# dfm/emcee

Hardware: AMD Instinct MI355X
Metric: walker-updates/sec (whole node), 64-dim correlated Gaussian, StretchMove a=2 (higher is better)
Workload: dtype f64

## Files before the change

emcee_amd/_lib.py:

```python
import ctypes as C
import os

import numpy as np

HERE = os.path.dirname(os.path.abspath(__file__))
LIB_PATH = os.path.join(HERE, "libemx.so")

TARGET_HOST, TARGET_ISO, TARGET_DIAG, TARGET_DENSE, TARGET_ROSENBROCK, TARGET_BOX, TARGET_CALLBACK = range(7)
TARGET_FUSED_USER = 8
TARGET_FUSED_PT = 9
TARGET_FUSED_ENSEMBLE = 10
MOVE_STRETCH, MOVE_DE, MOVE_SNOOKER, MOVE_GAUSS = range(4)
MOVE_WALK, MOVE_KDE = 5, 6
KDE_BW_SCOTT, KDE_BW_SILVERMAN, KDE_BW_SCALAR = range(3)
GAUSS_VECTOR, GAUSS_RANDOM, GAUSS_SEQUENTIAL = range(3)
RNG_INPUTS, RNG_MT19937, RNG_PHILOX = range(3)
EXCHANGE_ALLGATHER, EXCHANGE_PULL, EXCHANGE_DIRECT, EXCHANGE_LOGPROB, EXCHANGE_REPLAY = range(5)


class MoveDesc(C.Structure):
    _fields_ = [("kind", C.c_int32), ("nsplits", C.c_int32), ("randomize_split", C.c_int32), ("reserved", C.c_int32),
                ("a", C.c_double), ("sigma", C.c_double), ("g0", C.c_double), ("gammas", C.c_double)]


# ... 123 lines not shown
    "emx_logprob_finish": (C.c_int, [_P, C.c_int32]),
    "emx_replay_begin": (C.c_int, [_P, C.c_int32, C.POINTER(C.c_int64)]),
    "emx_replay_finish": (C.c_int, [_P, C.c_int32]),
    "emx_replay_exchange": (C.c_int, [_P, C.c_int32]),
    "emx_replica_pack": (C.c_int, [_P, C.POINTER(C.c_int64)]),
    "emx_replica_unpack": (C.c_int, [_P]),
    "emx_direct_export": (C.c_int, [_P, _u8p]),
    "emx_direct_import": (C.c_int, [_P, _u8p]),
    "emx_direct_attach": (C.c_int, [_P, C.POINTER(C.c_void_p), C.POINTER(C.c_void_p)]),
    "emx_direct_halfstep": (C.c_int, [_P, C.c_int32, C.c_int32]),
    "emx_fft_load": (C.c_int, [C.c_char_p]),
    "emx_autocorr": (C.c_int, [_P, C.c_int64, C.c_int64, C.c_double, _dp, _ip, C.POINTER(C.c_int64)]),
    "emx_walkers_independent": (C.c_int, [C.c_int32, _dp, C.c_int64, C.c_int32, C.POINTER(C.c_int32), C.POINTER(C.c_double)]),
    "emx_walkers_independent_resident": (C.c_int, [C.c_void_p, C.POINTER(C.c_int32), C.POINTER(C.c_double)]),
    "emx_host_pull_capacity": (C.c_int64, [C.c_int64, C.c_int32, C.c_int32, C.c_int32]),
    "emx_comm_load": (C.c_int, [C.c_char_p]),
    "emx_comm_get_unique_id": (C.c_int, [_u8p]),
    "emx_comm_init": (C.c_int, [_P, C.c_int32, C.c_int32, _u8p]),
    "emx_comm_destroy": (C.c_int, [_P]),
    "emx_comm_count": (C.c_int, [_P, C.POINTER(C.c_int32)]),
    "emx_pipeline_stats": (C.c_int, [_P, _dp, C.POINTER(C.c_int64), C.POINTER(C.c_int32)]),
    "emx_pipeline_handovers": (C.c_int, [_P, C.POINTER(C.c_int64), C.POINTER(C.c_int64)]),
    "emx_persist_info": (C.c_int, [_P, C.POINTER(C.c_int64)]),
    "emx_mtdev_info": (C.c_int, [_P, C.POINTER(C.c_int64)]),
    "emx_mtdev_debug": (C.c_int, [_P, C.c_int32, C.c_int64, C.c_void_p, C.c_int64]),
    "emx_mtdev_tok_stats": (C.c_int, [_P, C.POINTER(C.c_int64)]),
    "emx_persist_local_launches": (C.c_int, [_P, C.POINTER(C.c_int64)]),
    "emx_host_mt_jump": (C.c_int, [_u32p, C.c_uint64, C.c_int32, _u32p]),
    "emx_host_persist_shape": (C.c_int, [C.c_int64, C.c_int32, C.c_int32, C.POINTER(C.c_int32), C.POINTER(C.c_int32)]),
    "emx_timer_start": (C.c_int, [_P]),
    "emx_timer_stop": (C.c_int, [_P, C.POINTER(C.c_float)]),
    "emx_profile_enable": (C.c_int, [_P, C.c_int32]),
    "emx_profile_read": (C.c_int, [_P, _f32p, C.POINTER(C.c_int32)]),
    "emx_mt_create": (_P, [_u32p, C.c_int32, C.c_int32, C.c_double]),
    "emx_mt_destroy": (None, [_P]),
    "emx_mt_get_state": (None, [_P, _u32p, C.POINTER(C.c_int32), C.POINTER(C.c_int32), C.POINTER(C.c_double)]),
    "emx_mt_random_sample": (None, [_P, C.c_int64, _dp]),
    "emx_mt_randint": (None, [_P, C.c_uint64, C.c_int64, _i64p]),
    "emx_mt_randn": (None, [_P, C.c_int64, _dp]),
    "emx_mt_shuffle_labels": (None, [_P, C.c_int64, C.c_int32, _ip]),
    "emx_mt_choice_cdf": (C.c_int32, [_P, _dp, C.c_int32]),
    "emx_host_plan_mt": (C.c_int, [_P, C.c_int64, C.c_int32, C.POINTER(MoveDesc), _ip, _ip, _ip, _ip, _ip, _dp, _dp]),
    "emx_host_plan_mt_stream": (C.c_int, [_P, C.c_int64, C.c_int32, C.c_int32, C.POINTER(MoveDesc), _dp, C.c_int64, C.c_int32, C.c_int32,
                                          _P, _P, _P, _P, _P, _P, _P, C.POINTER(C.c_double)]),
    "emx_host_split_draws": (C.c_int, [_P, C.c_int64, C.POINTER(MoveDesc), _ip, _ip, C.c_int32, _ip, _ip, _ip, _dp]),
    "emx_host_plan_philox": (C.c_int, [C.c_uint64, C.c_uint64, C.c_int64, C.POINTER(MoveDesc), _ip, _ip, _ip, _ip, _ip, _dp, _dp]),
# ... 103 lines not shown
```

emcee_amd/csrc/emx.hip:

```cpp
#include <hip/hip_runtime.h>

#include <dlfcn.h>

#include <algorithm>
#include <chrono>
#include <cmath>
#include <cstdint>
#include <cstdio>
#include <cstring>
#include <deque>
#include <mutex>
#include <string>
#include <type_traits>
#include <vector>

#include "../../include/emx.h"
#include "emx_fused_ensemble.hpp"
#include "emx_fused_ensemble_data.hpp"
#include "emx_internal.hpp"
#include "emx_kernels.hpp"
#include "emx_launch.hpp"
#include "emx_mtdev.hpp"
#include "emx_mtjump.hpp"
#include "emx_mtpipe.hpp"
// ... 340 lines not shown
    int64_t tune_persist_slab_local_max = 4096;
    int64_t call_steps = 1;
    int64_t tune_persist_exact = 1;
    int64_t tune_persist_valu = 1;
    int64_t tune_persist_local_max = 8192;
    int64_t tune_slab = 1;
    int64_t tune_slab_skew = 1;
    int64_t tune_mt_device = 1;
    int64_t tune_mt_device_min = 147456;
    int64_t tune_mt_lookahead = 2;
    int64_t tune_mt_tok_wshift = 11, tune_mt_tok_tail = 2048;
    int64_t mtdev_steps_total = 0, mtdev_starts = 0;
    bool mtdev_defer_release = false;
    int64_t mtdev_release_pending = -1;
    MtDevStats mtdev_stats_last;
    int ring_pos = 0;
    struct Prepared {
        int move, S, slot;
        bool lean;
        int gcol;
        uint64_t step;
        NativeArgs nat;
        double cursor_before;
    };
    std::deque<Prepared> prepared;
    int64_t prep_hint = 1;
    std::vector<uint8_t> labels_scratch;
    struct Cur {
        bool active = false;
        int move = 0, S = 2, slot = 0;
        bool store = false;
        bool native = false;
        bool lean = false;
        bool devplan = false;
        int gcol = 0;
        std::vector<int32_t> off;
        NativeArgs nat{};
    } cur;
    double *chain = nullptr, *chain_lp = nullptr;
    int64_t cap = 0, stored = 0, proposals = 0;
    EnsSummary* summary = nullptr;
    RhatScratch* rhat = nullptr;
    int64_t tune_summary_compact = 1;
    int64_t tune_hist_chunk_rows = 0;
    double *qout = nullptr, *fout = nullptr, *newlp = nullptr;
    double* tp1_full = nullptr;
    double *evalX = nullptr, *evallp = nullptr;
    double* wk_work = nullptr;
// ... 90 lines not shown
    std::vector<hipEvent_t> prof;
    int prof_max = 0, prof_n = 0;
    std::string err;
    emx_fused_ensemble_data_fn fused_data_fn = nullptr;
    int64_t fused_ndata = 0;
    int64_t tune_fused_data_rows = 0;
};

static void graph_invalidate(emx_ctx* c);
static void apply_env_tuning(emx_ctx* c);
static int pipe_stop(emx_ctx* c);
#define PIPE_STOP(ctx)                        \
    do {                                      \
        const int _rps = pipe_stop(ctx);      \
        if (_rps) return _rps;                \
    } while (0)
static void direct_detach(emx_ctx* c);
static int direct_ensure(emx_ctx* c);
static void exchange_free(emx_ctx* c);
static int replay_ensure(emx_ctx* c);
static int flags_ensure(emx_ctx* c);
static int persist_settle(emx_ctx* c);
static hipError_t wait_stream(hipStream_t s);

static void drop_prepared(emx_ctx* c) {
    for (auto it = c->prepared.rbegin(); it != c->prepared.rend(); ++it)
        if (it->move < (int)c->moves.size() && c->moves[it->move].kind == EMX_MOVE_GAUSS) c->moves[it->move].gammas = it->cursor_before;
    c->prepared.clear();
}

#define FAIL(ctx, code, ...)                         \
    do {                                             \
        char _b[512];                                \
        snprintf(_b, sizeof(_b), __VA_ARGS__);       \
        if (ctx) (ctx)->err = _b; else g_err = _b;   \
        return (code);                               \
    } while (0)

#define HIPOK(ctx, expr)                                                                          \
    do {                                                                                          \
        hipError_t _e = (expr);                                                                   \
        if (_e != hipSuccess) FAIL(ctx, -2, "%s failed: %s (%s:%d)", #expr, hipGetErrorString(_e), __FILE__, __LINE__); \
    } while (0)

#define NEED(ctx, cond, ...)               \
    do {                                   \
// ... 732 lines not shown
}

static void apply_env_tuning(emx_ctx* c) {
    const char* e = getenv("EMX_TUNE");
    if (!e || !*e) return;
    std::string s(e);
    size_t pos = 0;
    while (pos < s.size()) {
        size_t end = s.find(',', pos);
        if (end == std::string::npos) end = s.size();
        const std::string kv = s.substr(pos, end - pos);
        const size_t eq = kv.find('=');
        if (eq != std::string::npos) emx_set_tuning(c, kv.substr(0, eq).c_str(), atoll(kv.c_str() + eq + 1));
        pos = end + 1;
    }
}

int emx_destroy(emx_ctx* c) {
    if (!c) return 0;
    pipe_stop(c);
    c->plog.clear();
    hipSetDevice(c->device);
    if (c->stream) hipStreamSynchronize(c->stream);
    if (c->comm && g_rccl.CommDestroy) g_rccl.CommDestroy(c->comm), c->comm = nullptr;
    if (c->status_host) hipHostFree(c->status_host);
    if (c->xfer_host) hipHostFree(c->xfer_host);
    for (int k = 0; k < 2; ++k) {
        if (c->bounce[k]) hipHostFree(c->bounce[k]);
        if (c->bounce_ev[k]) hipEventDestroy(c->bounce_ev[k]);
    }
    void* ptrs[] = {c->X, c->lp, c->acc, c->acc_count, c->iota, c->qout, c->fout, c->newlp, c->evalX, c->wk_work,
                    c->evallp, c->tp0, c->tp1, c->tp1_full, c->chain, c->chain_lp, c->own_shard_bufs ? c->sendbuf : nullptr,
                    c->own_shard_bufs ? c->gathered : nullptr};
    for (void* p : ptrs)
        if (p) hipFree(p);
    for (double* s : c->snap)
        if (s) hipFree(s);
    for (double* s : c->snap_blobs)
        if (s) hipFree(s);
    for (double* s : {c->blobs, c->evalblobs, c->blob_plane})
        if (s) hipFree(s);
    emx_internal_ens_summary_release(c->summary);
    emx_internal_rhat_release(c->rhat);

    for (auto& s : c->ring) {
        if (s.order) hipFree(s.order);
// ... 64 lines not shown
            const hipError_t e = hipStreamQuery(s);
            if (e != hipErrorNotReady) return e;
            if ((it & 63) == 63 && std::chrono::steady_clock::now() - t0 > std::chrono::milliseconds(2)) break;
        }
    }
    return hipStreamSynchronize(s);
}

static hipError_t wait_event(hipEvent_t ev) {
    if (g_spin_sync) {
        const auto t0 = std::chrono::steady_clock::now();
        for (int it = 0;; ++it) {
            const hipError_t e = hipEventQuery(ev);
            if (e != hipErrorNotReady) return e;
            if ((it & 63) == 63 && std::chrono::steady_clock::now() - t0 > std::chrono::milliseconds(2)) break;
        }
    }
    return hipEventSynchronize(ev);
}

int emx_sync(emx_ctx* c) {
    HIPOK(c, hipSetDevice(c->device));
    HIPOK(c, wait_stream(c->stream));
    return persist_settle(c);
}

int emx_status(emx_ctx* c, uint32_t* bits) {
    HIPOK(c, wait_stream(c->stream));
    {
        const int rcs = persist_settle(c);
        if (rcs) return rcs;
    }
    uint32_t b = 0;
    for (int k = 0; k < 6; ++k)
        if (__atomic_exchange_n(&c->status_host[k], 0u, __ATOMIC_ACQ_REL)) b |= 1u << k;
    if (b & ST_EXCHANGE_TIMEOUT) c->direct_dead = true;
    if (b & ST_EXCHANGE_TIMEOUT) c->persist_grid = 0;
    *bits = b;
    return 0;
}

int emx_set_tuning(emx_ctx* c, const char* key, int64_t v) {
    if (!strcmp(key, "spw")) {
        c->tune_spw = v;
        return 0;
    }
    if (!strcmp(key, "phase_clock")) {
// ... 153 lines not shown
        PIPE_STOP(c);
        c->tune_persist_exact = v ? 1 : 0;
        return 0;
    }
    if (!strcmp(key, "persist_exact_max_walkers")) {
        PIPE_STOP(c);
        c->tune_persist_exact_max = v;
        return 0;
    }
    if (!strcmp(key, "persist_exact_steps")) {
        c->tune_persist_exact_steps = std::max<int64_t>(1, std::min<int64_t>(v, 16));
        return 0;
    }
    if (!strcmp(key, "fetch_blocks")) {
        c->tune_fetch_blocks = std::max<int64_t>(0, std::min<int64_t>(v, 65536));
        return 0;
    }
    if (!strcmp(key, "fetch_avoid")) {
        c->tune_fetch_avoid = v ? 1 : 0;
        return 0;
    }
    if (!strcmp(key, "test_fetch_delay_us")) {
        c->tune_fetch_delay_us = std::max<int64_t>(0, std::min<int64_t>(v, 100000));
        return 0;
    }
    if (!strcmp(key, "persist_span")) {
        c->tune_persist_span = v ? 1 : 0;
        return 0;
    }
    if (!strcmp(key, "persist_mix")) {
        c->tune_persist_mix = v ? 1 : 0;
        return 0;
    }
    if (!strcmp(key, "persist_valu")) {
        c->tune_persist_valu = v ? 1 : 0;
        return 0;
    }
    if (!strcmp(key, "persist_local_max_walkers")) {
        c->tune_persist_local_max = v;
        return 0;
    }
    if (!strcmp(key, "persist_gauss_wpb")) {
        c->tune_persist_gauss_wpb = (v == 1 || v == 2 || v == 4 || v == 8) ? v : 0;
        return 0;
    }
    if (!strcmp(key, "persist_test_skew")) {
// ... 1065 lines not shown
    if (any_raw) hipLaunchKernelGGL(k_plan_raw_batch, dim3((unsigned)F.pieces_x, (unsigned)F.n), dim3(256), 0, c->up_stream, RB);
    HIPOK(c, hipGetLastError());
    hipEvent_t& ev = c->pipe_batch_ev[c->pipe_batch_n & 3];
    if (!ev) HIPOK(c, hipEventCreateWithFlags(&ev, hipEventDisableTiming));
    c->pipe_batch_n++;
    HIPOK(c, hipEventRecord(ev, c->up_stream));
    HIPOK(c, hipStreamWaitEvent(c->stream, ev, 0));
    for (auto& d : c->pipe_deferred) {
        c->ring[d.second].uploaded_ref = ev;
    }
    c->pipe_deferred.clear();
    return 0;
}

int emx_step_begin(emx_ctx* c, int32_t store, int32_t* move_out, int32_t* S_out) {
    return step_begin_impl(c, store, -1, move_out, S_out);
}

int emx_step_begin_with(emx_ctx* c, int32_t store, int32_t move_index, int32_t* S_out) {
    NEED(c, move_index >= 0 && move_index < (int)c->moves.size(), "bad move index");
    return step_begin_impl(c, store, move_index, nullptr, S_out);
}

static int native_prepare_batch(emx_ctx* c, uint64_t first_step, int nb, int forced_move, hipStream_t st) {
    const int nm = (int)c->moves.size();
    NativeBatchArgs B{};
    B.N = (int32_t)c->N;
    B.D = c->D;
    B.nb = nb;
    B.lean = (c->target != EMX_TARGET_HOST && c->world == 1 && !c->sendbuf && !c->comm && !c->tune_full_plan) ? 1 : 0;
    B.ablate = (int32_t)(c->tune_ablate >> 8);
    bool only_stretch = true;
    for (int b = 0; b < nb; ++b) {
        const uint64_t step = first_step + (uint64_t)b;
        const int mi = forced_move >= 0 ? forced_move : philox_move_choice(c->ph_seed, step, c->cdf.data(), nm);
        const emx_move_desc& m = c->moves[mi];
        only_stretch = only_stretch && m.kind == EMX_MOVE_STRETCH;
        emx_ctx::PlanSlot* ps;
        int rc = acquire_slot(c, &ps, false);
        if (rc) return rc;
        emx_ctx::Prepared pr{};
        pr.move = mi;
        pr.S = m.nsplits;
        pr.slot = c->ring_pos;
        pr.step = step;
        pr.nat.seed = c->ph_seed;
        pr.nat.step = step;
        pr.nat.pk = make_perm_key((uint64_t)c->N, c->ph_seed, step);
        pr.cursor_before = m.gammas;
        pr.lean = B.lean != 0;
        if (m.kind == EMX_MOVE_GAUSS) {
            B.gmode[b] = m.reserved;
            B.gcol[b] = (int32_t)((int64_t)m.gammas % c->D);
            pr.gcol = B.gcol[b];
            if (m.reserved == EMX_GAUSS_SEQUENTIAL) c->moves[mi].gammas = (double)(((int64_t)m.gammas + 1) % c->D);
        }
        c->prepared.push_back(pr);
        B.nat[b] = pr.nat;
        B.order[b] = ps->order;
        B.p0[b] = ps->p0;
        B.p1[b] = ps->p1;
        B.p2[b] = ps->p2;
        B.s0[b] = ps->s0;
        B.uacc[b] = ps->uacc;
        B.logu[b] = ps->logu;
        B.fac[b] = ps->fac;
        B.a[b] = m.a;
        B.sigma[b] = m.sigma;
        B.g0[b] = m.g0;
        B.move[b] = m.kind;
        B.S[b] = m.nsplits;
    }
    if (only_stretch && B.lean && !B.ablate && !B.desc)
        hipLaunchKernelGGL(k_native_plan_batch_stretch, dim3((unsigned)((c->N + 255) / 256), (unsigned)nb), dim3(256), 0, st, B);
    else
        hipLaunchKernelGGL(k_native_plan_batch, dim3((unsigned)((c->N + 255) / 256), (unsigned)nb), dim3(256), 0, st, B);
    HIPOK(c, hipGetLastError());
    return 0;
}

static int step_begin_impl(emx_ctx* c, int32_t store, int32_t forced_move, int32_t* move_out, int32_t* S_out) {
    HIPOK(c, hipSetDevice(c->device));
    NEED(c, !c->cur.active, "emx_step_begin: previous step not ended");
    if (store) NEED(c, c->stored < c->cap, "chain capacity exhausted (call emx_chain_config)");
    auto& cur = c->cur;
    cur.store = store != 0;
    cur.native = false;
    cur.devplan = false;
    const int nm = (int)c->moves.size();
    const bool devp = forced_move < 0 && mtdev_eligible(c);
    if (c->mtdev && !devp) {
        const int rcm = mtdev_stop(c);
        if (rcm) return rcm;
    }
    if (c->pipe && (devp || forced_move >= 0 || !pipe_eligible(c))) PIPE_STOP(c);
    if (devp) {
        if (!c->mtdev) {
            int rc0 = mtdev_start(c);
            if (rc0) return rc0;
        }
        int rc = mtdev_take(c);
        if (rc) return rc;
    } else if (c->rng_mode == EMX_RNG_MT19937 && forced_move < 0 && (c->pipe || ((c->N >= 8192 || persist_exact_ok(c)) && pipe_eligible(c)))) {
        if (!c->pipe) {
            int rc0 = pipe_start(c);
            if (rc0) return rc0;
        }
// ... 948 lines not shown
    const size_t lds = dense_lds_bytes(c->Dp, wpb);
    hipEvent_t e0 = nullptr, e1 = nullptr;
    const bool prof = c->prof_max > 0 && c->prof_n < c->prof_max;
    if (prof) {
        e0 = c->prof[2 * c->prof_n];
        e1 = c->prof[2 * c->prof_n + 1];
        HIPOK(c, hipEventRecord(e0, c->stream));
    }
    const hipError_t e = launch_hot_persist_gauss(c->Dp / 16, grid, block, lds, c->stream, P);
    if (e != hipSuccess) FAIL(c, -2, "persistent Gaussian launch failed: %s", hipGetErrorString(e));
    if (prof) {
        HIPOK(c, hipEventRecord(e1, c->stream));
        c->prof_n++;
    }
    c->persist_launches++;
    c->persist_halfsteps += steps;
    *done = steps;
    return 0;
}

static std::mutex g_persist_mu;
static hipEvent_t g_persist_ev[MAX_DEVICES] = {};
static const emx_ctx* g_persist_last[MAX_DEVICES] = {};

static int run_persist(emx_ctx* c, int64_t i0, int64_t total, int32_t thin_by, int32_t store, int64_t* done) {
    *done = 0;
    if (__atomic_load_n(&c->status_host[3], __ATOMIC_ACQUIRE)) {
        const int rcs = persist_settle(c);
        if (rcs) return rcs;
        if (__atomic_load_n(&c->status_host[3], __ATOMIC_ACQUIRE)) {
            c->persist_grid = 0;
            FAIL(c, -8, "persistent kernel: a device-wide barrier timed out in the middle of a launch; read emx_status, "
                        "or turn the persistent path off with tuning \"persist\" = 0");
        }
        return 0;
    }
    if (c->plog.size() >= 4096) {
        if (hipStreamQuery(c->stream) == hipSuccess && !__atomic_load_n(&c->status_host[3], __ATOMIC_ACQUIRE)) {
            c->plog.clear();
        } else if (c->plog.size() >= 65536) {
            const int rcs = persist_settle(c);
            if (rcs) return rcs;
        }
    }
    if (!c->persist_bar) {
        HIPOK(c, hipMalloc((void**)&c->persist_bar, PERSIST_BAR_WORDS * sizeof(unsigned)));
// ... 22 lines not shown
    } undefer2{c};
    c->mtdev_defer_release = devp;
    c->mtdev_release_pending = -1;
    struct Undefer {
        emx_ctx* c;
        ~Undefer() { c->mtdev_defer_release = false; }
    } undefer{c};
    emx_ctx::PersistLog lg{};
    lg.ph_step = c->ph_step;
    lg.i0 = i0;
    lg.stored0 = c->stored;
    lg.proposals0 = c->proposals;
    lg.thin_by = thin_by;
    lg.store = store;
    if (mtmode && !devp) {
        lg.pipe_step0 = c->pipe ? c->pipe_taken : 0;
        lg.pipe_id = c->pipe;
    }
    int launch_move = -1;
    int launch_S = 2;
    bool launch_local = false;
    bool launch_mix = false;
    double launch_gammas = 0.0;
    int batches_touched = (!mtmode && !c->prepared.empty() && c->prepared.front().step == c->ph_step) ? 1 : 0;
    while (i0 + steps < total) {
        if (!mtmode && (c->prepared.empty() || c->prepared.front().step != c->ph_step)) {
            if (batches_touched >= 2) break;
            ++batches_touched;
        }
        int next_move = -1;
        if (steps > 0 && !mtmode)
            next_move = !c->prepared.empty() ? c->prepared.front().move : philox_move_choice(c->ph_seed, c->ph_step, c->cdf.data(), (int)c->moves.size());
        if (steps > 0 && mtmode && !devp && c->moves.size() > 1) {
            PipeStepInfo peek;
            if (!c->pipe || !c->pipe->wait_ready(c->pipe_taken, peek, pipe_poll, c))
                FAIL(c, -7, "exact-mode plan pipeline stopped before step %lld", (long long)c->pipe_taken);
            next_move = peek.move;
        }
        int need = launch_S;
        if (launch_mix && next_move >= 0) need = c->moves[next_move].nsplits;
        if (n + need > (int)std::min<int64_t>(PERSIST_MAX_ITERS, std::max<int64_t>(4, c->tune_persist_max_halfsteps))) break;
        if (devp) {
            if (steps > 0 && c->mtdev && c->mtdev_taken % MTDEV_BATCH == 0) break;
        } else if (mtmode) {
            if (steps >= std::min<int64_t>(c->tune_persist_exact_steps, c->pipe_nsinks / 2)) break;
            if (steps > 0 && next_move >= 0) {
                if (!launch_mix && c->moves[next_move].kind != launch_move) break;
                if (!launch_mix && launch_move == EMX_MOVE_SNOOKER && c->moves[next_move].gammas != launch_gammas) break;
                if (launch_mix && !persist_mix_member(c->moves[next_move])) break;
                if (!persist_move_ok(c, c->moves[next_move])) break;
            }
// ... 1 lines not shown
            if (steps > 0 && c->prepared.empty() && !c->tune_persist_span) break;
            if (steps > 0 && !launch_mix && c->moves[next_move].kind != launch_move) break;
            if (steps > 0 && !launch_mix && launch_move == EMX_MOVE_SNOOKER && c->moves[next_move].gammas != launch_gammas) break;
            if (steps > 0 && launch_mix && !persist_mix_member(c->moves[next_move])) break;
            if (steps > 0 && !persist_move_ok(c, c->moves[next_move])) break;
        }
        c->prep_hint = NATIVE_BATCH_MAX;
        const int st = store && ((i0 + steps + 1) % thin_by == 0);
        int mvi, S;
        int rc = emx_step_begin(c, st, &mvi, &S);
        if (rc) return rc;
        if (launch_move < 0) {
            launch_move = c->moves[mvi].kind;
            launch_gammas = c->moves[mvi].gammas;
            launch_S = S;
            launch_local = persist_local_ok(c, c->moves[mvi]);
            c->persist_wpb = launch_local ? persist_shape_local_of(c->N, S, c->num_cu) : persist_shape(c, S);
            if (persist_mix_ok(c) && (launch_move == EMX_MOVE_DE || launch_move == EMX_MOVE_SNOOKER)) {
                launch_mix = true;
                launch_local = persist_mix_local(c);
                c->persist_wpb = launch_local ? persist_shape_local_of(c->N, 2, c->num_cu) : persist_shape(c, 2);
            }
        }
        for (int s = 0; s < S; ++s) {
            cap.got = false;
            c->persist_cap = &cap;
            rc = do_halfstep(c, s, c->target);
            c->persist_cap = nullptr;
            const bool valu = c->target != EMX_TARGET_DENSE_GAUSS;
            const bool move_ok = launch_mix ? (cap.move == MOVE_DE || cap.move == MOVE_SNOOKER) : cap.move == launch_move;
            if (!rc && (!cap.got || cap.dense == valu || (!valu && cap.dpb != c->Dp / 16) || !move_ok ||
                        (int)cap.block.x != 64 * c->persist_wpb || (valu && !launch_local && !persist_valu_wide_ok(c, c->moves[mvi])))) {
                c->err = "persistent half-steps: launch shape not eligible";
                rc = -1;
            }
            if (rc) {
                c->cur.active = false;
                return rc;
            }
            if (n == 0) {
                P.base = cap.a;
                grid = cap.grid;
                block = cap.block;
                lds = cap.lds;
            }
            PersistIter& I = P.it[n++];
            {
// ... 47 lines not shown
    P.timeout_ticks = 100000000ull * (unsigned long long)std::max<int64_t>(1, c->tune_persist_timeout_ms) / 1000ull;
    const bool fam_dense64 = c->target == EMX_TARGET_DENSE_GAUSS && c->Dp <= 64;
    P.stagger = c->tune_persist_stagger >= 0 ? (int32_t)c->tune_persist_stagger
                : (launch_local || store || !fam_dense64) ? 0
                : (launch_mix || launch_move == EMX_MOVE_DE) ? 528
                : launch_move == EMX_MOVE_STRETCH ? 516 : 0;
    c->persist_epoch += (unsigned)n;
    P.seq = ++c->persist_seq;
    lg.seq = P.seq;
    lg.steps = steps;
    if (!mtmode || (!devp && lg.pipe_id != nullptr)) c->plog.push_back(lg);
    hipEvent_t e0 = nullptr, e1 = nullptr;
    const bool prof = c->prof_max > 0 && c->prof_n < c->prof_max;
    if (prof) {
        e0 = c->prof[2 * c->prof_n];
        e1 = c->prof[2 * c->prof_n + 1];
    }
    {
        std::lock_guard<std::mutex> lk(g_persist_mu);
        const int dev = c->device;
        if (dev >= 0 && dev < MAX_DEVICES) {
            if (!g_persist_ev[dev]) HIPOK(c, hipEventCreateWithFlags(&g_persist_ev[dev], hipEventDisableTiming));
            if (g_persist_last[dev] && g_persist_last[dev] != c) HIPOK(c, hipStreamWaitEvent(c->stream, g_persist_ev[dev], 0));
        }
        if (prof) HIPOK(c, hipEventRecord(e0, c->stream));
        hipError_t e;
        const bool rows_late = store && (c->tune_persist_rows_late == 2 ||
                                         (c->tune_persist_rows_late == 1 && (launch_local || c->N / 2 / 16 >= 8 * (int64_t)c->num_cu)));
        if (c->target != EMX_TARGET_DENSE_GAUSS) {
            const Shape shv = pick_shape(c->D, c->D);
            e = launch_persist_valu(shv.G, shv.V, shv.CH, launch_move, launch_local ? 1 : 0, grid, block, c->stream, P);
        } else if (launch_mix) {
            e = launch_persist_mix(c->Dp / 16, launch_local ? 1 : 0, grid, block, lds, c->stream, P);
        } else if (c->Dp > 64) {
            P.base.ablate = c->tune_persist_slab_skew ? 256 | (int32_t)((c->tune_persist_slab_skew - 1) << 9) : 0;
            e = launch_persist_slab(c->Dp / 16, launch_move, launch_local ? 1 : 0, c->D & 1, grid, block, lds, c->stream, P);
            c->persist_slab_launches++;
        } else if (c->D & 1) {
            e = launch_persist_dense_odd(c->Dp / 16, launch_move, launch_local ? 1 : 0, grid, block, lds, c->stream, P);
        } else {
            e = launch_hot_persist_dense(c->Dp / 16, launch_move, launch_local ? 1 : 0, rows_late ? 1 : 0, grid, block, lds, c->stream, P);
        }
        if (launch_local) c->persist_local_launches++;
        if (e != hipSuccess) FAIL(c, -2, "persistent half-step launch failed: %s", hipGetErrorString(e));
        if (prof) {
            HIPOK(c, hipEventRecord(e1, c->stream));
            c->prof_n++;
// ... 176 lines not shown
int emx_small_info(emx_ctx* c, int64_t out[4]) {
    out[0] = c->small_launches;
    out[1] = c->small_steps;
    out[2] = out[3] = 0;
    return 0;
}

int emx_small_fused_pays(int64_t nwalkers, int32_t ndim, int32_t rng_mode) { return small_fused_pays(nwalkers, ndim, rng_mode) ? 1 : 0; }

int emx_small_fused_check(int64_t nwalkers, int32_t ndim, int32_t nmoves, const emx_move_desc* moves, int32_t rng_mode, int32_t nblobs,
                          char* msg, int32_t msglen) {
    char buf[320];
    const char* why = small_fused_refusal(nwalkers, ndim, nmoves, moves, rng_mode, nblobs, buf, sizeof buf);
    if (!why) return 0;
    if (msg && msglen > 0) snprintf(msg, (size_t)msglen, "%s", why);
    return -1;
}

int emx_persist_local_launches(emx_ctx* c, int64_t* n) {
    *n = c->persist_local_launches;
    return 0;
}

int emx_run(emx_ctx* c, int64_t nsteps, int32_t thin_by, int32_t store) {
    HIPOK(c, hipSetDevice(c->device));
    NEED(c, thin_by >= 1, "Invalid thinning argument");
    NEED(c, !c->cur.active, "emx_run: a step begun with emx_step_begin is still open");
    const int64_t total = nsteps * thin_by;
    c->call_steps = total;
    const bool devp = mtdev_eligible(c);
    if (c->mtdev && !devp) {
        const int rcm = mtdev_stop(c);
        if (rcm) return rcm;
    }
    const bool piped = !devp && pipe_eligible(c) && c->target != EMX_TARGET_HOST && (c->pipe || total >= 2);
    if (c->pipe && !piped) PIPE_STOP(c);
    if (c->pipe && persist_exact_ok(c) != (c->pipe_nsinks == PLAN_RING)) PIPE_STOP(c);
    if (piped && !c->pipe) {
        const int rc = pipe_start(c);
        if (rc) return rc;
    }
    const int rc = run_impl(c, nsteps, thin_by, store);
    c->call_steps = 1;
    if (rc && (c->pipe || c->mtdev)) pipe_stop(c);
    return rc;
}

static int run_impl(emx_ctx* c, int64_t nsteps, int32_t thin_by, int32_t store) {
    NEED(c, thin_by >= 1, "Invalid thinning argument");
    NEED(c, c->rng_mode != EMX_RNG_INPUTS, "emx_run needs an RNG mode that generates plans");
// ... 163 lines not shown
                }
                if (rc) {
                    c->cur.active = false;
                    return rc;
                }
            }
            rc = emx_step_end(c);
            if (rc) return rc;
            c->graph_warm = true;
            ctr_synced = false;
            ++i;
        }
    }
    c->prep_hint = 1;
    if (c->comm && (c->exchange == EMX_EXCHANGE_PULL || c->exchange == EMX_EXCHANGE_DIRECT) && c->world > 1) {
        int64_t per = 0;
        int rc = emx_replica_pack(c, &per);
        if (rc) return rc;
        const int e = g_rccl.AllGather(c->sendbuf, c->gathered, (size_t)per * (c->D + 3), RCCL_FLOAT64, c->comm, c->stream);
        if (e != 0) FAIL(c, -6, "ncclAllGather failed: %s", g_rccl.GetErrorString ? g_rccl.GetErrorString(e) : "?");
        rc = emx_replica_unpack(c);
        if (rc) return rc;
    }
    return 0;
}

static int64_t shard_rows_per_rank(int64_t N, int world, int min_nsplits = 2) {
    const int64_t maxns = (N + min_nsplits - 1) / min_nsplits + 1;
    return (maxns + world - 1) / world + 1;
}

static int min_nsplits_of(const emx_ctx* c) {
    int m = 2;
    for (const auto& mv : c->moves) m = std::min(m, (int)mv.nsplits);
    return std::max(1, m);
}

static int partners_of(int kind) {
    return kind == EMX_MOVE_GAUSS ? 0 : kind == EMX_MOVE_STRETCH ? 1 : kind == EMX_MOVE_DE ? 2 : 3;
}

static int64_t pull_capacity(int64_t N, int G, int S, int npart) {
    if (G <= 1) return 1;
    const int64_t bmax = (N + G - 1) / G, nsmax = (N + S - 1) / S;
    const int64_t hard = (int64_t)npart * std::min(bmax, nsmax);
    const double mean = (double)npart * (double)N / S / G / G;
// ... 1208 lines not shown
```

emcee_amd/device.py:

```python
import ctypes as C

import numpy as np

from . import _lib
from ._lib import EmxError, MoveDesc

__all__ = ["DeviceEnsemble", "EmxError"]

_STATUS_NAN_LOGP = 1
_STATUS_BAD_COORD = 2
_STATUS_EXCHANGE_OVERFLOW = 4
_STATUS_EXCHANGE_TIMEOUT = 8
_STATUS_PLAN_PRODUCER = 16
_STATUS_SINGULAR_COV = 32


def _blob_shape(b):
    return b[..., 0] if b.shape[-1] == 1 else b


def _as_f64(a, shape=None):
    a = np.ascontiguousarray(a, dtype=np.float64)
    if shape is not None and a.shape != shape:
        raise ValueError("expected array of shape %s, got %s" % (shape, a.shape))
# ... 611 lines not shown

    def pipeline_stats(self):
        out = np.zeros(6)
        n, k = C.c_int64(0), C.c_int32(0)
        self._ck(self.lib.emx_pipeline_stats(self.ctx, out, C.byref(n), C.byref(k)))
        if n.value <= 0:
            return None
        return {"steps_produced": n.value, "finisher_threads": k.value, "wall_us": out[0], "generator_us": out[1], "tokenizer_us": out[2],
                "finishers_us_summed": out[3], "tokenizer_waited_for_words_us": out[4], "tokenizer_waited_for_consumer_us": out[5]}

    def pipeline_handovers(self):
        raw, regen = C.c_int64(0), C.c_int64(0)
        self._ck(self.lib.emx_pipeline_handovers(self.ctx, C.byref(raw), C.byref(regen)))
        return {"raw_steps": int(raw.value), "regen_steps": int(regen.value)}

    def persist_info(self):
        out = (C.c_int64 * 4)()
        self._ck(self.lib.emx_persist_info(self.ctx, out))
        loc = C.c_int64(0)
        self._ck(self.lib.emx_persist_local_launches(self.ctx, C.byref(loc)))
        return {"qualifies": bool(out[0]), "launches": int(out[1]), "halfsteps": int(out[2]), "recovered": int(out[3]),
                "local_launches": int(loc.value)}

    def small_info(self):
        out = (C.c_int64 * 4)()
        self._ck(self.lib.emx_small_info(self.ctx, out))
        return {"launches": int(out[0]), "steps": int(out[1])}

    def mtdev_info(self):
        out = (C.c_int64 * 8)()
        self._ck(self.lib.emx_mtdev_info(self.ctx, out))
        return {"qualifies": bool(out[0]), "alive": bool(out[1]), "steps": int(out[2]), "rounds": int(out[3]), "segments": int(out[4]),
                "batches": int(out[5]), "windows": int(out[6]), "poly_us": int(out[7])}

    def mtdev_tok_stats(self):
        out = (C.c_int64 * 8)()
        self._ck(self.lib.emx_mtdev_tok_stats(self.ctx, out))
        return {"windows": int(out[0]), "rounds": int(out[1]), "tail_groups": int(out[2]), "tail_rounds": int(out[3]),
                "wait_us": out[4] / 100.0, "chunk_us": out[5] / 100.0, "tail_us": out[6] / 100.0, "kernel_us": out[7] / 100.0}

    def mtdev_debug(self, what, arg, n=0):
        if what == 0:
            out = np.empty(int(n), dtype=np.uint32)
        elif what == 1:
            out = np.empty(self.nwalkers, dtype=np.uint32)
        else:
# ... 26 lines not shown
```

include/emx.h:

```cpp
#ifndef EMX_H
#define EMX_H
#include <stdint.h>

#ifdef __cplusplus
extern "C" {
#endif

typedef struct emx_ctx emx_ctx;

enum emx_target_kind {
    EMX_TARGET_HOST = 0,
    EMX_TARGET_ISO_GAUSS = 1,
    EMX_TARGET_DIAG_GAUSS = 2,
    EMX_TARGET_DENSE_GAUSS = 3,
    EMX_TARGET_ROSENBROCK = 4,
    EMX_TARGET_BOX = 5,
    EMX_TARGET_DEVICE_CALLBACK = 6,
    EMX_TARGET_FUSED_USER = 8,
    EMX_TARGET_FUSED_PT = 9,
    EMX_TARGET_FUSED_ENSEMBLE = 10
};

enum emx_move_kind {
    EMX_MOVE_STRETCH = 0, EMX_MOVE_DE = 1, EMX_MOVE_SNOOKER = 2,
// ... 176 lines not shown
int emx_chain_minmax(emx_ctx* ctx, int32_t plane, int64_t start, int64_t stop, int64_t stride, double* lo_out, double* hi_out,
                     int64_t* nonfinite_out);
int emx_histograms(emx_ctx* ctx, int32_t plane, int64_t start, int64_t stop, int64_t stride, const int64_t* edge_off,
                   const double* edges, int64_t* counts_out, const int64_t* pedge_off, const double* pedges, int64_t npairs,
                   const int32_t* pairs, const int64_t* pair_off, int64_t* pair_counts_out, int64_t* nsamples_out);
int emx_walkers_independent(int32_t device, const double* coords, int64_t n, int32_t ndim, int32_t* independent,
                            double* cond_out);
int emx_walkers_independent_resident(emx_ctx* ctx, int32_t* independent, double* cond_out);

int emx_timer_start(emx_ctx* ctx);
int emx_timer_stop(emx_ctx* ctx, float* ms);
int emx_profile_enable(emx_ctx* ctx, int32_t max_launches);
int emx_profile_read(emx_ctx* ctx, float* ms_out, int32_t* n_inout);

int emx_pipeline_stats(emx_ctx* ctx, double out[6], int64_t* steps_produced, int32_t* finisher_threads);
int emx_pipeline_handovers(emx_ctx* ctx, int64_t* raw_steps, int64_t* regen_steps);

int emx_mtdev_info(emx_ctx* ctx, int64_t out[8]);
int emx_mtdev_debug(emx_ctx* ctx, int32_t what, int64_t arg, void* out, int64_t n);
int emx_mtdev_tok_stats(emx_ctx* ctx, int64_t out[8]);
int emx_host_mt_jump(const uint32_t key[624], uint64_t stride_words, int32_t k, uint32_t out_key[624]);

int emx_persist_info(emx_ctx* ctx, int64_t out[4]);
int emx_persist_local_launches(emx_ctx* ctx, int64_t* n);
int emx_host_persist_shape(int64_t nwalkers, int32_t nsplits, int32_t num_cu, int32_t* waves_per_group, int32_t* groups);

typedef struct emx_mt emx_mt;
emx_mt* emx_mt_create(const uint32_t key[624], int32_t pos, int32_t has_gauss, double cached);
void emx_mt_destroy(emx_mt* m);
void emx_mt_get_state(const emx_mt* m, uint32_t key[624], int32_t* pos, int32_t* has_gauss, double* cached);
void emx_mt_random_sample(emx_mt* m, int64_t n, double* out);
void emx_mt_randint(emx_mt* m, uint64_t bound, int64_t n, int64_t* out);
void emx_mt_randn(emx_mt* m, int64_t n, double* out);
void emx_mt_shuffle_labels(emx_mt* m, int64_t n, int32_t nsplits, int32_t* labels);
int32_t emx_mt_choice_cdf(emx_mt* m, const double* cdf, int32_t n);
int emx_host_plan_mt(emx_mt* m, int64_t nwalkers, int32_t ndim, const emx_move_desc* mv, int32_t* off, int32_t* order,
                     int32_t* p0, int32_t* p1, int32_t* p2, double* s0, double* uacc);
int emx_host_plan_mt_stream(emx_mt* m, int64_t nwalkers, int32_t ndim, int32_t nmoves, const emx_move_desc* moves,
                            const double* cdf, int64_t nsteps, int32_t nworkers, int32_t nsinks, int32_t* moves_out,
                            int32_t* order, int32_t* p0, int32_t* p1, int32_t* p2, double* s0, double* uacc,
                            double* seconds_out);
int emx_host_split_draws(emx_mt* m, int64_t nwalkers, const emx_move_desc* mv, const int32_t* off,
                         const int32_t* order, int32_t split, int32_t* p0, int32_t* p1, int32_t* p2, double* s0);
int emx_host_plan_philox(uint64_t seed, uint64_t step, int64_t nwalkers, const emx_move_desc* mv, int32_t* off,
                         int32_t* order, int32_t* p0, int32_t* p1, int32_t* p2, double* s0, double* uacc);
int32_t emx_host_move_choice_philox(uint64_t seed, uint64_t step, const double* cdf, int32_t n);
// ... 124 lines not shown
```

Before: 3.364 billion.

## Prepare next native plan batch ahead on a side stream after run

At the end of emx_run, the next batch of native step plans is enqueued on a separate non-blocking stream, ordered by events, so plan generation overlaps host idle time before the next call. The main stream waits on this work only if it has not finished. The persistent loop now tracks batch identity and can fill persistent iterations directly from the current native step without a halfstep call. This adds cross-context event ordering, a heuristic based on idle gaps, and timing instrumentation, at the cost of extra streams and events and more complex state.

```diff
diff --git a/emcee_amd/_lib.py b/emcee_amd/_lib.py
--- a/emcee_amd/_lib.py
+++ b/emcee_amd/_lib.py
@@ -169,6 +169,7 @@
     "emx_pipeline_stats": (C.c_int, [_P, _dp, C.POINTER(C.c_int64), C.POINTER(C.c_int32)]),
     "emx_pipeline_handovers": (C.c_int, [_P, C.POINTER(C.c_int64), C.POINTER(C.c_int64)]),
     "emx_persist_info": (C.c_int, [_P, C.POINTER(C.c_int64)]),
+    "emx_plan_ahead_info": (C.c_int, [_P, C.POINTER(C.c_int64)]),
     "emx_mtdev_info": (C.c_int, [_P, C.POINTER(C.c_int64)]),
     "emx_mtdev_debug": (C.c_int, [_P, C.c_int32, C.c_int64, C.c_void_p, C.c_int64]),
     "emx_mtdev_tok_stats": (C.c_int, [_P, C.POINTER(C.c_int64)]),
diff --git a/emcee_amd/csrc/emx.hip b/emcee_amd/csrc/emx.hip
--- a/emcee_amd/csrc/emx.hip
+++ b/emcee_amd/csrc/emx.hip
@@ -386,8 +386,22 @@
         uint64_t step;
         NativeArgs nat;
         double cursor_before;
+        unsigned batch;
     };
     std::deque<Prepared> prepared;
+    unsigned batch_seq = 0;
+    int64_t tune_plan_ahead = 1;
+    hipStream_t ahead_stream = nullptr;
+    hipEvent_t ahead_tail = nullptr, ahead_done = nullptr;
+    bool ahead_pending = false;
+    bool idle_seen = false;
+    std::chrono::steady_clock::time_point idle_t;
+    bool ahead_gap = true;
+    int ahead_hold = 0;
+    int64_t ahead_batches = 0;
+    std::chrono::steady_clock::time_point run_t0;
+    bool run_timing = false;
+    int64_t run_first_ns = -1, run_launch_ns = -1;
     int64_t prep_hint = 1;
     std::vector<uint8_t> labels_scratch;
     struct Cur {
@@ -524,6 +538,7 @@
 static int flags_ensure(emx_ctx* c);
 static int persist_settle(emx_ctx* c);
 static hipError_t wait_stream(hipStream_t s);
+static void ahead_release(emx_ctx* c);
 
 static void drop_prepared(emx_ctx* c) {
     for (auto it = c->prepared.rbegin(); it != c->prepared.rend(); ++it)
@@ -1302,6 +1317,7 @@
     c->plog.clear();
     hipSetDevice(c->device);
     if (c->stream) hipStreamSynchronize(c->stream);
+    ahead_release(c);
     if (c->comm && g_rccl.CommDestroy) g_rccl.CommDestroy(c->comm), c->comm = nullptr;
     if (c->status_host) hipHostFree(c->status_host);
     if (c->xfer_host) hipHostFree(c->xfer_host);
@@ -1412,7 +1428,10 @@
 int emx_sync(emx_ctx* c) {
     HIPOK(c, hipSetDevice(c->device));
     HIPOK(c, wait_stream(c->stream));
-    return persist_settle(c);
+    const int rc = persist_settle(c);
+    c->idle_seen = rc == 0;
+    c->idle_t = std::chrono::steady_clock::now();
+    return rc;
 }
 
 int emx_status(emx_ctx* c, uint32_t* bits) {
@@ -1612,6 +1631,11 @@
     }
     if (!strcmp(key, "test_fetch_delay_us")) {
         c->tune_fetch_delay_us = std::max<int64_t>(0, std::min<int64_t>(v, 100000));
+        return 0;
+    }
+    if (!strcmp(key, "plan_ahead")) {
+        NEED(c, v == 0 || v == 1, "tuning \"plan_ahead\" is 0 or 1");
+        c->tune_plan_ahead = v;
         return 0;
     }
     if (!strcmp(key, "persist_span")) {
@@ -2723,8 +2747,37 @@
     return step_begin_impl(c, store, move_index, nullptr, S_out);
 }
 
+static inline void run_mark_first(emx_ctx* c) {
+    if (c->run_timing && c->run_first_ns < 0)
+        c->run_first_ns = std::chrono::duration_cast<std::chrono::nanoseconds>(std::chrono::steady_clock::now() - c->run_t0).count();
+}
+
+static int ahead_join(emx_ctx* c, bool* waited = nullptr) {
+    if (!c->ahead_pending) return 0;
+    if (hipEventQuery(c->ahead_done) != hipSuccess) {
+        HIPOK(c, hipStreamWaitEvent(c->stream, c->ahead_done, 0));
+        if (waited) *waited = true;
+    }
+    c->ahead_pending = false;
+    return 0;
+}
+
+static bool plan_ahead_schedule_ok(const emx_ctx* c) {
+    if (c->rng_mode != EMX_RNG_PHILOX || c->target == EMX_TARGET_HOST) return false;
+    if (c->world != 1 || c->comm || c->sendbuf || c->peers_ready || c->tune_graph || c->tune_ablate || c->moves.empty()) return false;
+    for (const auto& m : c->moves)
+        if (m.kind != EMX_MOVE_STRETCH && m.kind != EMX_MOVE_DE && m.kind != EMX_MOVE_SNOOKER) return false;
+    return true;
+}
+
 static int native_prepare_batch(emx_ctx* c, uint64_t first_step, int nb, int forced_move, hipStream_t st) {
     const int nm = (int)c->moves.size();
+    if (st == c->stream) {
+        const int rcj = ahead_join(c);
+        if (rcj) return rcj;
+        run_mark_first(c);
+    }
+    const unsigned batch = ++c->batch_seq;
     NativeBatchArgs B{};
     B.N = (int32_t)c->N;
     B.D = c->D;
@@ -2749,6 +2802,7 @@
         pr.nat.step = step;
         pr.nat.pk = make_perm_key((uint64_t)c->N, c->ph_seed, step);
         pr.cursor_before = m.gammas;
+        pr.batch = batch;
         pr.lean = B.lean != 0;
         if (m.kind == EMX_MOVE_GAUSS) {
             B.gmode[b] = m.reserved;
@@ -2784,6 +2838,10 @@
     HIPOK(c, hipSetDevice(c->device));
     NEED(c, !c->cur.active, "emx_step_begin: previous step not ended");
     if (store) NEED(c, c->stored < c->cap, "chain capacity exhausted (call emx_chain_config)");
+    {
+        const int rcj = ahead_join(c);
+        if (rcj) return rcj;
+    }
     auto& cur = c->cur;
     cur.store = store != 0;
     cur.native = false;
@@ -3778,6 +3836,8 @@
 static std::mutex g_persist_mu;
 static hipEvent_t g_persist_ev[MAX_DEVICES] = {};
 static const emx_ctx* g_persist_last[MAX_DEVICES] = {};
+static hipEvent_t g_ahead_ev[MAX_DEVICES] = {};
+static const emx_ctx* g_ahead_last[MAX_DEVICES] = {};
 
 static int run_persist(emx_ctx* c, int64_t i0, int64_t total, int32_t thin_by, int32_t store, int64_t* done) {
     *done = 0;
@@ -3846,11 +3906,17 @@
     bool launch_local = false;
     bool launch_mix = false;
     double launch_gammas = 0.0;
-    int batches_touched = (!mtmode && !c->prepared.empty() && c->prepared.front().step == c->ph_step) ? 1 : 0;
+    int batches_touched = 0;
+    unsigned last_batch = 0;
     while (i0 + steps < total) {
-        if (!mtmode && (c->prepared.empty() || c->prepared.front().step != c->ph_step)) {
-            if (batches_touched >= 2) break;
-            ++batches_touched;
+        if (!mtmode) {
+            const bool fresh = c->prepared.empty() || c->prepared.front().step != c->ph_step;
+            const unsigned b = fresh ? c->batch_seq + 1 : c->prepared.front().batch;
+            if (b != last_batch) {
+                if (batches_touched >= 2) break;
+                ++batches_touched;
+                last_batch = b;
+            }
         }
         int next_move = -1;
         if (steps > 0 && !mtmode)
@@ -3898,7 +3964,21 @@
                 c->persist_wpb = launch_local ? persist_shape_local_of(c->N, 2, c->num_cu) : persist_shape(c, 2);
             }
         }
-        for (int s = 0; s < S; ++s) {
+        const bool direct = steps > 0 && !mtmode && !launch_mix && S == launch_S && c->moves[mvi].kind == launch_move && c->cur.native &&
+                            c->cur.slot >= 0 && n + S <= PERSIST_MAX_ITERS;
+        for (int s = 0; direct && s < S; ++s) {
+            const auto& cur = c->cur;
+            PersistIter& I = P.it[n++];
+            I.plan = reinterpret_cast<const char*>(c->ring[cur.slot].order);
+            I.chain = cur.store ? c->chain + (size_t)c->stored * c->N * c->D : nullptr;
+            I.chain_lp = cur.store ? c->chain_lp + (size_t)c->stored * c->N : nullptr;
+            I.pos0 = cur.off[s];
+            I.split = s;
+            I.kind = c->moves[mvi].kind;
+            I.gammas = c->moves[mvi].gammas;
+            I.shift = 0;
+        }
+        for (int s = 0; !direct && s < S; ++s) {
             cap.got = false;
             c->persist_cap = &cap;
             rc = do_halfstep(c, s, c->target);
@@ -3992,7 +4072,11 @@
         if (dev >= 0 && dev < MAX_DEVICES) {
             if (!g_persist_ev[dev]) HIPOK(c, hipEventCreateWithFlags(&g_persist_ev[dev], hipEventDisableTiming));
             if (g_persist_last[dev] && g_persist_last[dev] != c) HIPOK(c, hipStreamWaitEvent(c->stream, g_persist_ev[dev], 0));
-        }
+            if (g_ahead_last[dev] && g_ahead_last[dev] != c) HIPOK(c, hipStreamWaitEvent(c->stream, g_ahead_ev[dev], 0));
+        }
+        run_mark_first(c);
+        if (c->run_timing && c->run_launch_ns < 0)
+            c->run_launch_ns = std::chrono::duration_cast<std::chrono::nanoseconds>(std::chrono::steady_clock::now() - c->run_t0).count();
         if (prof) HIPOK(c, hipEventRecord(e0, c->stream));
         hipError_t e;
         const bool rows_late = store && (c->tune_persist_rows_late == 2 ||
@@ -4215,10 +4299,92 @@
     return 0;
 }
 
+static int plan_ahead_topup(emx_ctx* c) {
+    if (!c->tune_plan_ahead || !plan_ahead_schedule_ok(c) || !c->ahead_gap || c->cur.active || c->ahead_pending) return 0;
+    if (!c->prepared.empty() && c->prepared.front().step != c->ph_step) drop_prepared(c);
+    if (c->prepared.size() >= (size_t)NATIVE_BATCH_MAX) return 0;
+    if (c->ahead_hold > 0) {
+        --c->ahead_hold;
+        return 0;
+    }
+    if (!c->ahead_stream) {
+        HIPOK(c, hipStreamCreateWithFlags(&c->ahead_stream, hipStreamNonBlocking));
+        HIPOK(c, hipEventCreateWithFlags(&c->ahead_tail, hipEventDisableTiming));
+        HIPOK(c, hipEventCreateWithFlags(&c->ahead_done, hipEventDisableTiming));
+    }
+    HIPOK(c, hipEventRecord(c->ahead_tail, c->stream));
+    HIPOK(c, hipStreamWaitEvent(c->ahead_stream, c->ahead_tail, 0));
+    const int dev = c->device;
+    if (dev >= 0 && dev < MAX_DEVICES) {
+        std::lock_guard<std::mutex> lk(g_persist_mu);
+        if (g_persist_last[dev] && g_persist_last[dev] != c && g_persist_ev[dev]) HIPOK(c, hipStreamWaitEvent(c->ahead_stream, g_persist_ev[dev], 0));
+        if (g_ahead_last[dev] && g_ahead_last[dev] != c) HIPOK(c, hipStreamWaitEvent(c->ahead_stream, g_ahead_ev[dev], 0));
+    }
+    const uint64_t first = c->prepared.empty() ? c->ph_step : c->prepared.back().step + 1;
+    const int rc = native_prepare_batch(c, first, NATIVE_BATCH_MAX, -1, c->ahead_stream);
+    if (rc) return rc;
+    HIPOK(c, hipEventRecord(c->ahead_done, c->ahead_stream));
+    (void)hipEventQuery(c->ahead_tail);
+    (void)hipStreamQuery(c->ahead_stream);
+    c->ahead_pending = true;
+    c->ahead_batches++;
+    if (dev >= 0 && dev < MAX_DEVICES) {
+        std::lock_guard<std::mutex> lk(g_persist_mu);
+        g_ahead_ev[dev] = c->ahead_done;
+        g_ahead_last[dev] = c;
+    }
+    return 0;
+}
+
+static void ahead_release(emx_ctx* c) {
+    if (!c->ahead_stream) return;
+    hipStreamSynchronize(c->ahead_stream);
+    if (c->device >= 0 && c->device < MAX_DEVICES) {
+        std::lock_guard<std::mutex> lk(g_persist_mu);
+        if (g_ahead_last[c->device] == c) {
+            g_ahead_last[c->device] = nullptr;
+            g_ahead_ev[c->device] = nullptr;
+        }
+    }
+    if (c->ahead_tail) hipEventDestroy(c->ahead_tail);
+    if (c->ahead_done) hipEventDestroy(c->ahead_done);
+    hipStreamDestroy(c->ahead_stream);
+    c->ahead_stream = nullptr;
+    c->ahead_tail = c->ahead_done = nullptr;
+    c->ahead_pending = false;
+}
+
+int emx_plan_ahead_info(emx_ctx* c, int64_t out[5]) {
+    out[0] = c->ahead_batches;
+    out[1] = (c->tune_plan_ahead && plan_ahead_schedule_ok(c)) ? 1 : 0;
+    out[2] = c->run_first_ns;
+    out[3] = c->run_launch_ns;
+    out[4] = (c->ahead_pending && hipEventQuery(c->ahead_done) == hipErrorNotReady) ? 1 : 0;
+    return 0;
+}
+
 int emx_run(emx_ctx* c, int64_t nsteps, int32_t thin_by, int32_t store) {
     HIPOK(c, hipSetDevice(c->device));
     NEED(c, thin_by >= 1, "Invalid thinning argument");
     NEED(c, !c->cur.active, "emx_run: a step begun with emx_step_begin is still open");
+    c->run_t0 = std::chrono::steady_clock::now();
+    c->run_first_ns = c->run_launch_ns = -1;
+    c->run_timing = true;
+    struct RunTimed {
+        emx_ctx* c;
+        ~RunTimed() { c->run_timing = false; }
+    } run_timed{c};
+    {
+        if (c->idle_seen)
+            c->ahead_gap = c->run_t0 - c->idle_t >= std::chrono::microseconds(20);
+        else
+            c->ahead_gap = !(c->tune_plan_ahead && plan_ahead_schedule_ok(c) && hipStreamQuery(c->stream) == hipErrorNotReady);
+        c->idle_seen = false;
+        bool waited = false;
+        const int rcj = ahead_join(c, &waited);
+        if (rcj) return rcj;
+        if (waited) c->ahead_hold = 8;
+    }
     const int64_t total = nsteps * thin_by;
     c->call_steps = total;
     const bool devp = mtdev_eligible(c);
@@ -4428,6 +4594,7 @@
         rc = emx_replica_unpack(c);
         if (rc) return rc;
     }
+    if (total > 0 && !small_on && !persist_gauss_on) return plan_ahead_topup(c);
     return 0;
 }
 
diff --git a/emcee_amd/device.py b/emcee_amd/device.py
--- a/emcee_amd/device.py
+++ b/emcee_amd/device.py
@@ -657,6 +657,13 @@
         return {"qualifies": bool(out[0]), "launches": int(out[1]), "halfsteps": int(out[2]), "recovered": int(out[3]),
                 "local_launches": int(loc.value)}
 
+    def plan_ahead_info(self):
+        out = (C.c_int64 * 5)()
+        self._ck(self.lib.emx_plan_ahead_info(self.ctx, out))
+        us = [None if int(v) < 0 else int(v) / 1e3 for v in (out[2], out[3])]
+        return {"batches": int(out[0]), "enabled": bool(out[1]), "first_enqueue_us": us[0], "persist_launch_us": us[1],
+                "in_flight": bool(out[4])}
+
     def small_info(self):
         out = (C.c_int64 * 4)()
         self._ck(self.lib.emx_small_info(self.ctx, out))
diff --git a/include/emx.h b/include/emx.h
--- a/include/emx.h
+++ b/include/emx.h
@@ -222,6 +222,7 @@
 int emx_host_mt_jump(const uint32_t key[624], uint64_t stride_words, int32_t k, uint32_t out_key[624]);
 
 int emx_persist_info(emx_ctx* ctx, int64_t out[4]);
+int emx_plan_ahead_info(emx_ctx* ctx, int64_t out[5]);
 int emx_persist_local_launches(emx_ctx* ctx, int64_t* n);
 int emx_host_persist_shape(int64_t nwalkers, int32_t nsplits, int32_t num_cu, int32_t* waves_per_group, int32_t* groups);
 
diff --git a/profiles/r07/trace_digest.py b/profiles/r07/trace_digest.py
--- /dev/null
+++ b/profiles/r07/trace_digest.py
@@ -0,0 +1,24 @@
+import csv
+import glob
+import sys
+
+d, tag = sys.argv[1], sys.argv[2]
+files = glob.glob(d + "/**/*kernel_trace.csv", recursive=True)
+rows = []
+for f in files:
+    for r in csv.DictReader(open(f)):
+        rows.append((int(r["Start_Timestamp"]), int(r["End_Timestamp"]), r["Kernel_Name"]))
+rows.sort()
+tail = rows[-14:]
+t0 = tail[0][0]
+print("## %s: the last %d kernels of the run (the timed call is the last k_persist launch)" % (tag, len(tail)))
+print("start_us  dur_us  idle_before_us  kernel")
+prev_end = None
+for s, e, name in tail:
+    short = name.split("(")[0][-70:]
+    print("%9.1f %7.1f %9s  %s" % ((s - t0) / 1e3, (e - s) / 1e3, "-" if prev_end is None else "%.1f" % ((s - prev_end) / 1e3), short))
+    prev_end = e
+durs = [(e - s) / 1e3 for s, e, n in rows if "k_persist" in n and (e - s) > 300e3]
+if durs:
+    durs.sort()
+    print("k_persist launches longer than 300 us: n=%d median %.1f us min %.1f max %.1f" % (len(durs), durs[len(durs) // 2], durs[0], durs[-1]))
```

After: 3.307 billion. -1.7%, worse.
